# awslabs/crowd-coachable-recommendations

Measured on AMD Instinct MI355X. Metric: queries/sec, exhaustive inner-product top-100 retrieval (NQ-shaped 2,681,468 x 768 bf16 corpus), higher is better.
Workload: dtype bf16

## Files before the change

crowd-coachable-recommendations_amd/ccrec_amd/_lib.py:

```python
import ctypes
import os

_HERE = os.path.dirname(os.path.abspath(__file__))
LIB_PATH = os.path.join(os.path.dirname(_HERE), "lib", "libccr_hip.so")

CCR_OK = 0
CCR_ERR_INVALID, CCR_ERR_HIP, CCR_ERR_WORKSPACE, CCR_ERR_BLOCK_ID = -1, -2, -3, -4
DTYPE_F32, DTYPE_F16, DTYPE_BF16 = 0, 1, 2
SEARCH_DEFAULT, SEARCH_FORCE_DENSE, SEARCH_FORCE_FUSED, SEARCH_ASYNC = 0, 1, 2, 4
SCORES_CANONICAL, SCORES_MFMA = 0, 1

EXPORTS = [
    "ccr_last_error", "ccr_version", "ccr_pack_bf16", "ccr_pack_bf16_ex", "ccr_meanpool_pack_bf16", "ccr_meanpool_pack_bf16_ex", "ccr_index_create",
    "ccr_index_create_with_norms", "ccr_index_destroy",
    "ccr_index_rows", "ccr_index_dim", "ccr_search_workspace_bytes", "ccr_search", "ccr_search_last_stats",
    "ccr_merge_topk", "ccr_merge_topk_strided", "ccr_apply_block", "ccr_inbatch_ce_workspace_bytes", "ccr_inbatch_ce_fwd", "ccr_inbatch_ce_bwd", "ccr_inbatch_ce_bwd_dev", "ccr_rank_metrics",
    "ccr_search_finish", "ccr_scores", "ccr_search_blocked_workspace_bytes", "ccr_search_blocked",
    "ccr_search_sparse_prior_workspace_bytes", "ccr_search_sparse_prior", "ccr_colsum_bf16", "ccr_meanpool_bwd", "ccr_bm25_index_create", "ccr_bm25_index_destroy", "ccr_bm25_search_workspace_bytes",
    "ccr_bm25_search", "ccr_pack_bf16_padded", "ccr_shard_message_bytes", "ccr_search_shard", "ccr_shard_message_fill", "ccr_merge_shard_messages",
    "ccr_attention_bf16", "ccr_add_layernorm", "ccr_meanpool_pack_bf16_packed", "ccr_embed_layernorm", "ccr_gelu_bf16",
    "ccr_attention_half", "ccr_add_layernorm_half", "ccr_embed_layernorm_half", "ccr_gelu_half", "ccr_merge_short_lists",
    "ccr_bm25_search_workspace_bytes_k", "ccr_bm25_search_last_stats", "ccr_bm25_index_set_idf", "ccr_inbatch_pack3_bf16", "ccr_inbatch_ce_fwd_f32",
    "ccr_search_stream_wait_main_pass", "ccr_pool_ce_workspace_bytes", "ccr_pool_ce_fwd", "ccr_pool_ce_fwd_f32", "ccr_pool_ce_bwd_dev",
    "ccr_bpr_sample", "ccr_bpr_frozen_workspace_bytes", "ccr_bpr_frozen_fwd", "ccr_bpr_frozen_bwd_dev",
    "ccr_attention_fwd_train_half", "ccr_attention_bwd_workspace_bytes", "ccr_attention_bwd_half", "ccr_add_layernorm_bwd_half", "ccr_gelu_bwd_half",
    "ccr_dropout_bits_rows", "ccr_dropout_bits_attention", "ccr_dropout_apply", "ccr_attention_fwd_train_drop_half", "ccr_attention_bwd_drop_half",
    "ccr_add_layernorm_drop_half", "ccr_add_layernorm_bwd_drop_half",
]

MIN_VERSION = 101
BPR_VERSION = 102
ENCODER_TRAIN_VERSION = 103
ENCODER_DROPOUT_VERSION = 104

SHARD_HEADER_BYTES = 32
SHARD_MAGIC = 0x4D524343


class ShardHeader(ctypes.Structure):
    _fields_ = [("magic", ctypes.c_uint32), ("n_flagged", ctypes.c_uint32), ("k_valid", ctypes.c_uint32),
                ("n_covered", ctypes.c_uint32), ("row_offset", ctypes.c_int64), ("n_rows", ctypes.c_int64)]


class SearchStats(ctypes.Structure):
    _fields_ = [("path", ctypes.c_int32), ("n_fallback", ctypes.c_int32), ("sample_tiles", ctypes.c_int32),
                ("ranges", ctypes.c_int32), ("cap", ctypes.c_int32), ("sublists", ctypes.c_int32),
                ("n_candidates", ctypes.c_int64), ("ms_sample", ctypes.c_float), ("ms_threshold", ctypes.c_float),
                ("ms_main", ctypes.c_float), ("ms_select", ctypes.c_float), ("ms_fallback", ctypes.c_float),
                ("ms_total", ctypes.c_float), ("n_retried", ctypes.c_int32), ("n_dense", ctypes.c_int32),
                ("main_launches", ctypes.c_int32), ("opt_rank", ctypes.c_int32), ("main_tile_queries", ctypes.c_int32),
                ("skipped_tiles", ctypes.c_int32)]


class CcrError(RuntimeError):
    pass


_lib = None


def load():
    global _lib
    if _lib is not None:
        return _lib
    if not os.path.isfile(LIB_PATH):
        raise CcrError(f"{LIB_PATH} not built: run `python -c 'import __graft_entry__ as g; g.build()'` "
# ... 18 lines not shown
    lib.ccr_meanpool_pack_bf16_ex.argtypes = [vp, i32, vp, vp, vp, vp, vp, i32, i32, i32, i32, vp]
    lib.ccr_index_create.argtypes = [vp, i64, i32, i64, vp, ctypes.POINTER(vp)]
    lib.ccr_index_destroy.argtypes = [vp]
    lib.ccr_index_rows.argtypes = [vp]
    lib.ccr_index_rows.restype = i64
    lib.ccr_index_dim.argtypes = [vp]
    lib.ccr_search_workspace_bytes.argtypes = [vp, i32, i32]
    lib.ccr_search_workspace_bytes.restype = sz
    lib.ccr_search.argtypes = [vp, vp, i32, i32, vp, vp, vp, sz, i32, vp]
    lib.ccr_search_last_stats.argtypes = [vp, ctypes.POINTER(SearchStats)]
    lib.ccr_merge_topk.argtypes = [vp, vp, i32, i32, i32, vp, vp, vp]
    lib.ccr_merge_topk_strided.argtypes = [vp, vp, i64, i64, i32, i32, i32, vp, vp, vp]
    lib.ccr_apply_block.argtypes = [vp, vp, i32, i32, vp, vp, i64, vp, vp, i32, vp]
    lib.ccr_inbatch_ce_workspace_bytes.argtypes = [i32, i32]
    lib.ccr_inbatch_ce_workspace_bytes.restype = sz
    lib.ccr_inbatch_ce_fwd.argtypes = [vp, vp, vp, i32, i32, f32, vp, vp, vp, sz, vp]
    lib.ccr_inbatch_ce_bwd.argtypes = [vp, vp, vp, vp, i32, i32, f32, f32, vp, vp, vp, vp, sz, vp]
    lib.ccr_inbatch_ce_bwd_dev.argtypes = [vp, vp, vp, vp, i32, i32, f32, vp, vp, vp, vp, vp, sz, vp]
    lib.ccr_inbatch_pack3_bf16.argtypes = [vp, vp, vp, i32, i32, vp, vp]
    lib.ccr_inbatch_ce_fwd_f32.argtypes = [vp, vp, vp, i32, i32, f32, vp, vp, vp, vp, sz, vp]
    lib.ccr_pool_ce_workspace_bytes.argtypes = [i32, i32, i32]
    lib.ccr_pool_ce_workspace_bytes.restype = sz
    lib.ccr_pool_ce_fwd.argtypes = [vp, vp, vp, vp, i32, i32, i32, f32, vp, vp, vp, sz, vp]
    lib.ccr_pool_ce_fwd_f32.argtypes = [vp, vp, vp, vp, i32, i32, i32, f32, vp, vp, vp, vp, sz, vp]
    lib.ccr_pool_ce_bwd_dev.argtypes = [vp, vp, vp, vp, vp, i32, i32, i32, f32, vp, vp, vp, vp, vp, sz, vp]
    lib.ccr_bpr_sample.argtypes = [vp, i32, i32, i64, vp, vp, vp, f32, vp, vp, i32, vp, i32, vp, vp]
    lib.ccr_bpr_frozen_workspace_bytes.argtypes = [i32, i32, i32]
    lib.ccr_bpr_frozen_workspace_bytes.restype = sz
    lib.ccr_bpr_frozen_fwd.argtypes = [vp, i64, i32, vp, vp, f32, vp, vp, vp, vp, i32, i32, vp, vp, sz, vp]
    lib.ccr_bpr_frozen_bwd_dev.argtypes = [vp, i64, i32, vp, vp, f32, vp, vp, vp, vp, i32, i32, vp, vp, vp, vp, vp, sz, vp]
    lib.ccr_rank_metrics.argtypes = [vp, i32, i32, vp, vp, vp, i32, vp, vp, vp]
    lib.ccr_search_finish.argtypes = [vp]
    lib.ccr_search_stream_wait_main_pass.argtypes = [vp, vp]
    lib.ccr_scores.argtypes = [vp, vp, i32, i32, vp, vp]
    lib.ccr_search_blocked_workspace_bytes.argtypes = [vp, i32, i32, vp]
    lib.ccr_search_blocked_workspace_bytes.restype = sz
    lib.ccr_search_blocked.argtypes = [vp, vp, i32, i32, vp, vp, vp, vp, vp, sz, i32, vp]
    lib.ccr_search_sparse_prior_workspace_bytes.argtypes = [vp, i32, i32, vp]
    lib.ccr_search_sparse_prior_workspace_bytes.restype = sz
    lib.ccr_search_sparse_prior.argtypes = [vp, vp, i32, i32, vp, vp, vp, vp, vp, vp, sz, i32, vp]
    lib.ccr_colsum_bf16.argtypes = [vp, i64, i32, vp, vp]
    lib.ccr_meanpool_bwd.argtypes = [vp, vp, vp, i32, i32, i32, i32, vp]
    lib.ccr_bm25_index_create.argtypes = [vp, vp, vp, vp, i64, i64, ctypes.c_double, ctypes.POINTER(vp)]
    lib.ccr_bm25_index_destroy.argtypes = [vp]
    lib.ccr_bm25_search_workspace_bytes.argtypes = [vp, i32, i32]
    lib.ccr_bm25_search_workspace_bytes.restype = sz
    lib.ccr_bm25_search_workspace_bytes_k.argtypes = [vp, i32, i32, i32]
    lib.ccr_bm25_search_workspace_bytes_k.restype = sz
    lib.ccr_bm25_search_last_stats.argtypes = [vp, vp]
    lib.ccr_bm25_index_set_idf.argtypes = [vp, vp, vp, vp]
    lib.ccr_bm25_search.argtypes = [vp, vp, vp, vp, i32, i32, vp, vp, vp, sz, vp]
    lib.ccr_pack_bf16_padded.argtypes = [vp, i64, i32, vp, i32, vp, vp, i32, vp]
    lib.ccr_attention_bf16.argtypes = [vp, vp, vp, vp, i32, i32, i32, i32, ctypes.c_float, vp]
    lib.ccr_add_layernorm.argtypes = [vp, vp, vp, vp, ctypes.c_float, vp, vp, i64, i32, vp]
    lib.ccr_embed_layernorm.argtypes = [vp, i64, vp, i64, vp, i64, vp, vp, vp, vp, vp, ctypes.c_float, vp, vp, i64, i32, vp]
    lib.ccr_gelu_bf16.argtypes = [vp, vp, i64, vp]
    lib.ccr_attention_half.argtypes = [vp, vp, vp, vp, i32, i32, i32, i32, ctypes.c_float, i32, vp]
    lib.ccr_add_layernorm_half.argtypes = [vp, vp, vp, vp, ctypes.c_float, vp, vp, i64, i32, i32, vp]
    lib.ccr_embed_layernorm_half.argtypes = [vp, i64, vp, i64, vp, i64, vp, vp, vp, vp, vp, ctypes.c_float, vp, vp, i64, i32, i32, vp]
    lib.ccr_gelu_half.argtypes = [vp, vp, i64, i32, vp]
    lib.ccr_attention_fwd_train_half.argtypes = [vp, vp, vp, vp, vp, i32, i32, i32, i32, ctypes.c_float, i32, vp]
    lib.ccr_attention_bwd_workspace_bytes.argtypes = [i32, i32, i32]
    lib.ccr_attention_bwd_workspace_bytes.restype = sz
    lib.ccr_attention_bwd_half.argtypes = [vp, vp, vp, vp, vp, vp, vp, i32, i32, i32, i32, ctypes.c_float, i32, vp, sz, vp]
    lib.ccr_add_layernorm_bwd_half.argtypes = [vp, vp, vp, ctypes.c_float, vp, vp, vp, vp, vp, i64, i32, i32, vp, sz, vp]
    lib.ccr_gelu_bwd_half.argtypes = [vp, vp, vp, i64, i32, vp]
# ... 30 lines not shown
```

crowd-coachable-recommendations_amd/ccrec_amd/ops.py:

```python
import contextlib
import ctypes

import torch

from . import _lib

_DTYPES = {torch.float32: _lib.DTYPE_F32, torch.float16: _lib.DTYPE_F16, torch.bfloat16: _lib.DTYPE_BF16}


def require_gpu():
    if not torch.cuda.is_available():
        raise _lib.CcrError("ccrec_amd needs a ROCm GPU (torch.cuda.is_available() is False); there is no CPU fallback")
    return _lib.load()


def _stream(t):
    return ctypes.c_void_p(torch.cuda.current_stream(t.device).cuda_stream)


def _ptr(t):
    return ctypes.c_void_p(t.data_ptr()) if t is not None else None


_NO_SWITCH = contextlib.nullcontext()
# ... 697 lines not shown
        return scores, ids

    def search_sparse_prior(self, queries_bf16, k, prior_ptr, prior_idx, prior_val, flags=_lib.SEARCH_DEFAULT):
        q, ptr, idx = self._special_args(queries_bf16, prior_ptr, prior_idx)
        val = torch.as_tensor(prior_val, dtype=torch.float64).to(q.device).contiguous()
        assert val.numel() == idx.numel()
        n_q = q.shape[0]
        scores = torch.empty(n_q, k, dtype=torch.float64, device=q.device)
        ids = torch.empty(n_q, k, dtype=torch.int64, device=q.device)
        if n_q == 0:
            return scores, ids
        if n_q > MAX_QUERIES_PER_SEARCH:
            for lo in range(0, n_q, MAX_QUERIES_PER_SEARCH):
                hi = min(n_q, lo + MAX_QUERIES_PER_SEARCH)
                a, b = int(ptr[lo]), int(ptr[hi])
                s_part, i_part = self.search_sparse_prior(q[lo:hi], k, ptr[lo:hi + 1] - a, idx[a:b], val[a:b], flags)
                scores[lo:hi], ids[lo:hi] = s_part, i_part
            return scores, ids
        pp = ctypes.c_void_p(ptr.data_ptr())
        need = int(self._lib.ccr_search_sparse_prior_workspace_bytes(self._h, n_q, k, pp))
        if need == 0:
            raise _lib.CcrError("ccr_search_sparse_prior: " + self._lib.ccr_last_error().decode("utf-8", "replace"))
        ws = self._special_ws(need)
        with _on(q):
            _lib.check(self._lib.ccr_search_sparse_prior(self._h, _ptr(q), n_q, k, pp, _ptr(idx), _ptr(val), _ptr(scores),
                                                         _ptr(ids), _ptr(ws), ws.numel(), int(flags), _stream(q)),
                       "ccr_search_sparse_prior")
        return scores, ids

    def last_stats(self):
        st = _lib.SearchStats()
        _lib.check(self._lib.ccr_search_last_stats(self._h, ctypes.byref(st)), "ccr_search_last_stats")
        return {f: getattr(st, f) for f, _ in st._fields_}

    def scores(self, queries_bf16, mode="canonical"):
        q = queries_bf16.contiguous()
        assert q.is_cuda and q.dtype == torch.bfloat16 and q.dim() == 2 and q.shape[1] == self.dim
        out = torch.empty(q.shape[0], self.n_rows, dtype=torch.float32, device=q.device)
        if q.shape[0] == 0:
            return out
        m = {"canonical": _lib.SCORES_CANONICAL, "mfma": _lib.SCORES_MFMA}[mode]
        with _on(q):
            _lib.check(self._lib.ccr_scores(self._h, _ptr(q), q.shape[0], m, _ptr(out), _stream(q)), "ccr_scores")
        return out


def _rank_strided(t):
    return t.dim() == 3 and t.stride(2) == 1 and t.stride(1) == t.shape[2] and t.stride(0) >= t.shape[1] * t.shape[2]


def merge_topk(scores, ids):
    lib = require_gpu()
    assert scores.is_cuda and scores.dtype == torch.float32 and ids.dtype == torch.int64 and scores.shape == ids.shape
    if not _rank_strided(scores):
        scores = scores.contiguous()
    if not _rank_strided(ids):
        ids = ids.contiguous()
    R, n_q, k = scores.shape
    os_ = torch.empty(n_q, k, dtype=torch.float32, device=scores.device)
    oi = torch.empty(n_q, k, dtype=torch.int64, device=scores.device)
    with _on(scores):
        _lib.check(lib.ccr_merge_topk_strided(_ptr(scores), _ptr(ids), scores.stride(0), ids.stride(0), R, n_q, k, _ptr(os_),
                                              _ptr(oi), _stream(scores)), "ccr_merge_topk")
    return os_, oi


# ... 347 lines not shown
```

crowd-coachable-recommendations_amd/csrc/ccr_api.hip:

```cpp
#include <stdarg.h>
#include <stdlib.h>
#include <string.h>

#include <math.h>

#include <algorithm>
#include <mutex>
#include <vector>

#include "ccr_index.h"
#include "ccr_narrow.h"
#include "ccr_topk_device.h"

namespace ccr {

static thread_local char g_err[512] = "";
void set_error(const char *fmt, ...) {
    va_list ap;
    va_start(ap, fmt);
    vsnprintf(g_err, sizeof(g_err), fmt, ap);
    va_end(ap);
}

static int env_int(const char *name, int dflt) {
    const char *e = getenv(name);
    return e ? atoi(e) : dflt;
}

Knobs read_knobs() {
    Knobs kn;
    kn.qgroups = env_int("CCR_QGROUPS", 0);
    kn.progressive = env_int("CCR_PROGRESSIVE", 1);
    kn.max_phases = env_int("CCR_PHASES", 3);
    kn.mfma16 = env_int("CCR_MFMA16", -1);
    kn.sample_div = env_int("CCR_SAMPLE_DIV", 0);
    kn.max_lists = env_int("CCR_MAX_LISTS", 0);
    kn.ranges = env_int("CCR_RANGES", 0);
    kn.optimistic = env_int("CCR_OPTIMISTIC", -1);
    kn.opt_rank = env_int("CCR_OPT_RANK", 0);
    kn.narrow = env_int("CCR_NARROW", -1);
    kn.wide = env_int("CCR_WIDE", -1);
    kn.skip_sampled = env_int("CCR_SKIP_SAMPLED", -1);
    kn.skip_list = env_int("CCR_SKIP_LIST", 1);
    kn.narrow_grid = env_int("CCR_NARROW_GRID", 0);
    kn.narrow_groups = env_int("CCR_NARROW_GROUPS", NARROW_MAX_GROUPS);
    return kn;
}

static int pick_qgroups(int qblocks, int dim, const Knobs &kn, int tile_q = TILE_Q) {
    {
        const int v = kn.qgroups;
        if ((v == 1 || v == 2 || v == 4 || v == 8) && qblocks % v == 0) return v;
    }
    const size_t block_bytes = (size_t)tile_q * dim * 2;
    int best = 1;
    for (int gq = 1; gq <= NUM_XCD; gq *= 2) {
        if (qblocks % gq) continue;
        best = gq;
        if ((size_t)(qblocks / gq) * block_bytes <= (size_t)3 << 20) break;
    }
    return best;
}

static inline int64_t round_up(int64_t v, int64_t m) { return (v + m - 1) / m * m; }

static int best_sample_ranges(int64_t n_vt, int qblocks, int qgroups, int grid) {
    const int nrc = NUM_XCD / qgroups, qb_per = qblocks / qgroups, per_x = std::max(1, grid / NUM_XCD);
    int best_r = NUM_XCD;
    double best = 1e300;
    const int64_t r_max = round_up(std::min<int64_t>(n_vt, 1024), NUM_XCD);
    std::vector<double> load((size_t)per_x);
    for (int64_t R = NUM_XCD; R <= r_max; R += NUM_XCD) {
        double worst = 0.0;
        for (int rc = 0; rc < nrc; ++rc) {
            std::fill(load.begin(), load.end(), 0.0);
            const int64_t items = R / nrc * qb_per;
            for (int64_t item = 0; item < items; ++item) {
                const int64_t r = rc + nrc * (item / qb_per);
                const int64_t ntile = (n_vt - r + R - 1) / R;
                if (ntile > 0) load[(size_t)(item % per_x)] += (double)ntile + 0.15;
            }
            worst = std::max(worst, *std::max_element(load.begin(), load.end()));
        }
        if (worst < best - 1e-9) {
            best = worst;
            best_r = (int)R;
        }
    }
    return best_r;
}

constexpr size_t DENSE_SCRATCH_TARGET = (size_t)1 << 30;

struct MainPassChoice {
// ... 157 lines not shown
                            narrow_lds_bytes(nqt, dim) <= (size_t)160 * 1024 && (ngroups == 1 || num_cu >= 16);
        p.narrow = narrow ? nqt : 0;
        p.narrow_groups = narrow ? ngroups : 1;
        p.tile_q = TILE_Q;
        p.main_qblocks = p.qblocks;
        if (!narrow && p.mfma16 && dim % 32 == 0 && kn.wide != 0) {
            const int wb = (n_q + WIDE_Q - 1) / WIDE_Q;
            const double per_xcd = (double)(wb / pick_qgroups(wb, dim, kn, WIDE_Q)) * WIDE_Q * dim * 2.0;
            const double per_flop = per_xcd <= 3.2 * 1048576.0 ? 0.95 : (per_xcd <= 5.5 * 1048576.0 ? 0.97 : 1.04);
            if (kn.wide == 1 || (double)wb * WIDE_Q * per_flop < (double)p.qblocks * TILE_Q) {
                p.tile_q = WIDE_Q;
                p.main_qblocks = wb;
                p.nq_pad = (int)round_up(std::max<int64_t>(n_q, (int64_t)wb * WIDE_Q), TILE_Q);
                p.qblocks = p.nq_pad / TILE_Q;
                p.qgroups = pick_qgroups(p.qblocks, dim, kn);
            }
        }
        p.main_qgroups = pick_qgroups(p.main_qblocks, dim, kn, p.tile_q);
        MainPassChoice choice = choose_main_pass(p, k, sample, sample_alt, sample_big, kn, narrow);
        if (choice.opt_rank > 0 && may_skip_sampled(p, choice.sample, narrow, kn)) {
            const MainPassChoice skipped = choose_main_pass(p, k, sample, sample_alt, sample_big, kn, narrow, choice.sample);
            if (skipped.skip) choice = skipped;
        }
        sample = choice.sample;
        const int64_t R = choice.ranges;
        p.sample_tiles = (int)sample;
        p.sample_stride = std::max<int64_t>(1, p.full_tiles / sample);
        p.sample_ranges = best_sample_ranges(sample, p.qblocks, p.qgroups, p.grid);
        p.ranges = (int)R;
        p.item_a = choice.item_a;
        p.item_b = choice.item_b;
        p.opt_rank = choice.opt_rank;
        p.skip_sampled = (p.opt_rank > 0 && !p.narrow) ? choice.skip : 0;
        if (p.skip_sampled) {
            const double join_rows = 256.0 * (double)choice.sample * (1.0 - pow(1.0 - std::min(1.0, (double)k / (double)n_rows), 16.0));
            const double need = (double)k + (double)(k / 4) + 1.5 * join_rows + TILE_DOCS + 16;
            const double saved = 0.5 * (double)choice.sample * p.main_qblocks * (p.tile_q == WIDE_Q ? 1.37 : 1.0) / (double)p.grid;
            const bool pays = 0.065 * join_rows * ((double)p.nq_pad / 3584.0) < saved;
            if (need > 8192.0 || (kn.skip_sampled < 0 && !pays))
                p.skip_sampled = 0;
            else
                p.rescore_cap = std::min(8192, std::max(p.rescore_cap, pow2_ceil((int)need)));
        }
        const int nrc_p = NUM_XCD / p.main_qgroups, qb_per_p = p.main_qblocks / p.main_qgroups;
        const int64_t RA = p.item_a ? std::min<int64_t>(R, (int64_t)nrc_p * ((p.item_a + qb_per_p - 1) / qb_per_p)) : 0;
        const int64_t RB = p.item_b ? std::min<int64_t>(R, (int64_t)nrc_p * ((p.item_b + qb_per_p - 1) / qb_per_p)) : 0;
        const double ratio = (double)p.tiles / (double)sample;
        const double expect = (double)k * ratio * 1.3 + 64.0;
        const double fs = 1.0 / ratio, nlists = (double)R * p.sublists;
        const double xk = 1.25 * ((double)k + 4.75 * sqrt((double)k) + 8.0) / (double)k;
        const int64_t tile_rows = TILE_DOCS / p.sublists;
        const double xr = p.opt_rank ? 1.25 * ((double)p.opt_rank + 4.75 * sqrt((double)p.opt_rank) + 8.0) / (double)p.opt_rank : 0.0;
        auto cap_for = [&](double g) -> int {
            const double mean = p.opt_rank ? xr * std::max((double)p.opt_rank / fs, (double)k) / nlists : xk * (double)k / (g * nlists);
            const int64_t c = (int64_t)(mean + 6.0 * sqrt(mean)) + 16 + tile_rows;
            return (int)round_up(std::min<int64_t>(std::max<int64_t>(c, 16), 8192), 4);
        };
        const double fa = p.item_a ? (double)(p.item_a / qb_per_p) * nrc_p / (double)R : 0.0;
        const double fb = p.item_b ? std::max(0.0, (double)(p.item_b / qb_per_p) * nrc_p / (double)R - fa) : 0.0;
        const double upd_compact = std::min(32768.0, std::max(4096.0, 8.0 * pow2_ceil(k)));
        auto seen = [&](double g, double found) { return found > upd_compact ? g * upd_compact / found : g; };
        const double found_a = (double)k * fa / fs;
        CandLayout &L = p.cand;
        memset(&L, 0, sizeof(L));
        const int seg_end_v[3] = {RA ? (int)RA : (int)R, RB > RA ? (int)RB : (int)R, (int)R};
        int64_t recs = 0;
// ... 121 lines not shown
int slab_take(int device, uint32_t **out, volatile uint32_t **host_out) {
    std::lock_guard<std::mutex> lock(g_slab_mutex);
    CCR_REQUIRE(device >= 0 && device < MAX_DEVICES, "device ordinal %d out of range", device);
    Slab &sl = g_slabs[device];
    if (!sl.base) {
        CCR_HIP_CHECK(hipMalloc((void **)&sl.base, (size_t)SLAB_SLOTS * SLAB_SLOT_BYTES));
        if (hipHostMalloc((void **)&sl.host, (size_t)SLAB_SLOTS * SLAB_HOST_BYTES, hipHostMallocDefault) != hipSuccess) {
            (void)hipFree(sl.base);
            sl.base = nullptr;
            set_error("ccr_index_create: hipHostMalloc of the pinned flag lines failed");
            return CCR_ERR_HIP;
        }
        for (int i = SLAB_SLOTS - 1; i >= 0; --i) sl.free_slots.push_back(i);
    }
    if (sl.free_slots.empty()) {
        set_error("ccr_index_create: more than %d live indices on device %d", SLAB_SLOTS, device);
        return CCR_ERR_INVALID;
    }
    *out = reinterpret_cast<uint32_t *>(sl.base + (size_t)sl.free_slots.back() * SLAB_SLOT_BYTES);
    *host_out = reinterpret_cast<volatile uint32_t *>(sl.host + (size_t)sl.free_slots.back() * SLAB_HOST_BYTES);
    sl.free_slots.pop_back();
    return CCR_OK;
}

void slab_give(int device, uint32_t *p) {
    if (!p || device < 0 || device >= MAX_DEVICES) return;
    std::lock_guard<std::mutex> lock(g_slab_mutex);
    Slab &sl = g_slabs[device];
    sl.free_slots.push_back((int)((reinterpret_cast<char *>(p) - sl.base) / SLAB_SLOT_BYTES));
}
}

extern "C" const char *ccr_last_error(void) { return g_err; }
extern "C" int ccr_version(void) { return 104; }

extern "C" int ccr_index_destroy(ccr_index *ix);

namespace {
struct CachedBlock {
    void *p;
    size_t bytes;
};
std::vector<CachedBlock> g_blocks[MAX_DEVICES];
constexpr size_t BLOCK_CACHE_ENTRIES = 8;

int block_take(int device, size_t bytes, void **out, size_t *got) {
    CCR_REQUIRE(device >= 0 && device < MAX_DEVICES, "device ordinal %d out of range", device);
    bytes = (bytes + 4095) / 4096 * 4096;
    {
        std::lock_guard<std::mutex> lock(g_slab_mutex);
        auto &v = g_blocks[device];
        for (size_t i = 0; i < v.size(); ++i)
            if (v[i].bytes >= bytes && v[i].bytes <= 2 * bytes) {
                *out = v[i].p;
                *got = v[i].bytes;
                v.erase(v.begin() + i);
                return CCR_OK;
            }
    }
    CCR_HIP_CHECK(hipMalloc(out, bytes));
    *got = bytes;
    return CCR_OK;
}

void block_give(int device, void *p, size_t bytes) {
    if (!p) return;
    void *drop = nullptr;
// ... 84 lines not shown
    block_give(ix->device, ix->row_norm_own, ix->row_bytes);
    if (ix->have_events)
        for (int i = 0; i < EV_COUNT; ++i)
            if (ix->ev[i]) (void)hipEventDestroy(ix->ev[i]);
    delete ix;
    return CCR_OK;
}

extern "C" int64_t ccr_index_rows(const ccr_index *ix) { return ix ? ix->n_rows : -1; }
extern "C" int ccr_index_dim(const ccr_index *ix) { return ix ? ix->dim : -1; }

extern "C" size_t ccr_search_workspace_bytes(const ccr_index *ix, int n_q, int k) {
    if (!ix || n_q <= 0 || k <= 0) return 0;
    Plan a = make_plan(ix->n_rows, ix->dim, n_q, k, CCR_SEARCH_DEFAULT, ix->num_cu, ix->knobs);
    Plan b = make_plan(ix->n_rows, ix->dim, n_q, k, CCR_SEARCH_FORCE_DENSE, ix->num_cu, ix->knobs);
    Plan c = make_plan(ix->n_rows, ix->dim, n_q, k, CCR_SEARCH_FORCE_FUSED, ix->num_cu, ix->knobs);
    return std::max({a.total, b.total, c.total}) + 256;
}

extern "C" int ccr_search_stream_wait_main_pass(const ccr_index *ix, void *stream) {
    CCR_REQUIRE(ix, "ccr_search_stream_wait_main_pass: null index");
    if (!ix->main_pass_recorded) return CCR_OK;
    CCR_HIP_CHECK(hipStreamWaitEvent((hipStream_t)stream, ix->ev[EV_MAIN_END], 0));
    return CCR_OK;
}

extern "C" int ccr_search_last_stats(const ccr_index *ix, ccr_search_stats *stats) {
    CCR_REQUIRE(ix && stats, "ccr_search_last_stats: null pointer");
    CCR_REQUIRE(!ix->pending.active, "ccr_search_last_stats: an asynchronous search is pending (call ccr_search_finish first)");
    *stats = ix->stats;
    return CCR_OK;
}

static int dense_for_list(const ccr_index *ix, const uint16_t *Q, const uint32_t *d_qlist, int n, int k, float *scratch, int64_t rows_per_chunk,
                          float *out_scores, int64_t *out_ids, hipStream_t s) {
    for (int lo = 0; lo < n; lo += (int)rows_per_chunk) {
        const int m = std::min<int64_t>(rows_per_chunk, n - lo);
        int rc = launch_dense_scores(ix->D, ix->n_rows, ix->dim, Q, d_qlist ? d_qlist + lo : nullptr, lo, m, nullptr, scratch, s);
        if (rc != CCR_OK) return rc;
        rc = launch_dense_select(scratch, ix->n_rows, k, d_qlist ? d_qlist + lo : nullptr, lo, m, nullptr, ix->id_out, out_scores, out_ids, s);
        if (rc != CCR_OK) return rc;
    }
    return CCR_OK;
}

static bool margin_path_ok(const ccr_index *ix, int k) { return ix->dim % 8 == 0 && k <= MAX_K; }
static int64_t tiles_of(const ccr_index *ix) { return (ix->n_rows + TILE_DOCS - 1) / TILE_DOCS; }

static GemmArgs gemm_args(const ccr_index *ix, const uint16_t *Q, int n_q, int nq_pad) {
    GemmArgs g;
    memset(&g, 0, sizeof(g));
    g.D = ix->D;
    g.n_rows = ix->n_rows;
    g.dim = ix->dim;
    g.Q = Q;
    g.n_q = n_q;
    g.nq_pad = nq_pad;
    g.qblocks = nq_pad / TILE_Q;
    g.item_end = INT32_MAX;
    return g;
}

static GemmArgs filter_args(const ccr_index *ix, const Plan &p, const SearchWs &w, const uint16_t *Q, int n_q, int nq_pad, int qblocks,
                            int qgroups, const float *thr, const float *cq, const CandLayout &lay) {
    GemmArgs g = gemm_args(ix, Q, n_q, nq_pad);
    g.qblocks = qblocks;
// ... 12 lines not shown

static int store_scores(const ccr_index *ix, const uint16_t *Q, int n_q, int ranges, float *out, int64_t pitch, hipStream_t s) {
    GemmArgs g = gemm_args(ix, Q, n_q, (int)round_up(n_q, TILE_Q));
    g.n_vt = tiles_of(ix);
    g.tile_stride = 1;
    g.ranges = ranges;
    g.qgroups = 1;
    g.store = out;
    g.store_pitch = pitch;
    return launch_gemm(g, ix->knobs.mfma16 != 0 ? MAIN_16X16 : MAIN_32X32, EPI_STORE, std::max(NUM_XCD, ix->num_cu / NUM_XCD * NUM_XCD), s);
}

static int margin_for_rows(const ccr_index *ix, const uint16_t *Qc, const float *hint, const uint32_t *out_rows, int n, int k, float *scratch,
                           size_t scratch_bytes, float *out_scores, int64_t *out_ids, uint32_t *flag_count, uint32_t *flag_list, hipStream_t s) {
    const int64_t pitch = round_up(ix->n_rows, 4);
    int64_t chunk = (int64_t)(scratch_bytes / ((size_t)pitch * 4));
    CCR_REQUIRE(chunk >= 1, "margin path: no room for one score row");
    if (chunk > TILE_Q) chunk = chunk / TILE_Q * TILE_Q;
    const int ranges = (int)round_up(std::min<int64_t>(std::max<int64_t>(1, tiles_of(ix) / 4), 1024), NUM_XCD);
    for (int lo = 0; lo < n; lo += (int)chunk) {
        const int m = std::min<int64_t>(chunk, n - lo);
        const uint16_t *Q = Qc + (int64_t)lo * ix->dim;
        int rc = store_scores(ix, Q, m, ranges, scratch, pitch, s);
        if (rc != CCR_OK) return rc;
        rc = launch_margin_select(scratch, pitch, ix->n_rows, k, ix->dim, Q, ix->D, ix->tile_norm, ix->row_norm, ix->dmax_bits,
                                  hint ? hint + lo : nullptr, out_rows ? out_rows + lo : nullptr, lo, m, ix->id_out, out_scores, out_ids, flag_count, flag_list, s);
        if (rc != CCR_OK) return rc;
    }
    return CCR_OK;
}

static int run_main_pass(const ccr_index *ix, const Plan &p, const SearchWs &w, const uint16_t *Q, int n_q, int k, hipStream_t s) {
    GemmArgs gm = filter_args(ix, p, w, Q, n_q, p.nq_pad, p.main_qblocks, p.main_qgroups, w.thr, w.cq, p.cand);
    if (p.skip_sampled) {
        gm.n_vt = p.tiles - p.sample_tiles;
        gm.skip_stride = (int)p.sample_stride;
        gm.skip_count = p.sample_tiles;
    }
    const int nrc = NUM_XCD / gm.qgroups, qb_per = gm.qblocks / gm.qgroups, items = p.ranges / nrc * qb_per;
    const int bounds[4] = {0, p.item_a, p.item_b, items};
    int done = 0, updates = 0, prev_full = 0, prev_part = 0, prev_blocks = 0;
    for (int ph = 1; ph < 4; ++ph) {
        if (bounds[ph] <= done) continue;
        if (done > 0) {
            const int rl_full = done / qb_per, part = done % qb_per;
            const int full = rl_full * nrc * p.sublists, partial = part ? (rl_full + 1) * nrc * p.sublists : 0;
            const bool more = bounds[ph] < items && ph < 3;
            const int rc = launch_threshold_update(w.cand, w.cnt, full, partial, part, prev_full, prev_part, prev_blocks, qb_per, p.sublists, n_q,
                                                   p.nq_pad, p.cand, k, w.cq, ix->tile_norm, p.item_b ? w.top : nullptr, updates > 0, more, w.thr, s, p.tile_q);
            if (rc != CCR_OK) return rc;
            prev_full = full;
            prev_part = partial;
            prev_blocks = part;
            ++updates;
        }
        gm.item_begin = done;
        gm.item_end = bounds[ph];
        const MainKernel kind = p.tile_q == WIDE_Q ? MAIN_WIDE : p.mfma16 ? MAIN_16X16 : MAIN_32X32;
        const int rc = launch_gemm(gm, kind, EPI_FILTER, p.grid, s);
        if (rc != CCR_OK) return rc;
        done = bounds[ph];
    }
    return CCR_OK;
}

static int run_narrow_pass(const ccr_index *ix, const Plan &p, const SearchWs &w, const uint16_t *Q, int n_q, hipStream_t s) {
// ... 346 lines not shown
```

crowd-coachable-recommendations_amd/csrc/ccr_common.h:

```cpp
#pragma once
#include <hip/hip_runtime.h>
#include <stdint.h>
#include <stdio.h>

#include "ccr_retrieval.h"

namespace ccr {

void set_error(const char *fmt, ...);

#define CCR_HIP_CHECK(expr)                                                                   \
    do {                                                                                      \
        hipError_t _e = (expr);                                                               \
        if (_e != hipSuccess) {                                                               \
            ccr::set_error("%s failed: %s (%s:%d)", #expr, hipGetErrorString(_e), __FILE__, __LINE__); \
            return CCR_ERR_HIP;                                                               \
        }                                                                                     \
    } while (0)

#define CCR_REQUIRE(cond, ...)            \
    do {                                  \
        if (!(cond)) {                    \
            ccr::set_error(__VA_ARGS__);  \
            return CCR_ERR_INVALID;       \
// ... 15 lines not shown
constexpr int TILE_K = 32;
constexpr int GEMM_THREADS = 512;
constexpr int GROUPS_PER_TILE = 16;
constexpr int MAX_K = 4096;
constexpr uint32_t FLAG_DENSE = 0x80000000u;
constexpr int NUM_XCD = 8;

struct CandLayout {
    int nseg;
    int seg_end[3];
    int cap[3];
    long long base[3];
};
__host__ __device__ __forceinline__ void cand_segment(const CandLayout &L, int r, int &cap, int &r0, long long &base) {
    const int g = (r >= L.seg_end[0] ? 1 : 0) + (r >= L.seg_end[1] ? 1 : 0);
    r0 = g ? L.seg_end[g - 1] : 0;
    cap = L.cap[g];
    base = L.base[g];
}
__host__ __device__ __forceinline__ long long cand_sublist(const CandLayout &L, int r, int q, int s, int nq_pad, int sp, int &cap) {
    const int g = (r >= L.seg_end[0] ? 1 : 0) + (r >= L.seg_end[1] ? 1 : 0);
    const int r0 = g ? L.seg_end[g - 1] : 0;
    cap = L.cap[g];
    return L.base[g] + (((long long)(r - r0) * nq_pad + q) * sp) * (long long)cap + s;
}

struct Plan {
    int fused;
    int nq_pad;
    int qblocks;
    int tile_q;
    int main_qblocks;
    int main_qgroups;
    int64_t tiles;
    int64_t full_tiles;
    int sample_tiles;
    int64_t sample_stride;
    int sample_ranges;
    int ranges;
    int item_a;
    int item_b;
    int opt_rank;
    int skip_sampled;
    int qgroups;
    int cap;
    CandLayout cand;
    int grid;
    int rescore_cap;
    int rescore_regular;
    int select_compact;
    int mfma16;
    int sublists;
    int narrow;
    int narrow_groups;
    int first_nsub;
    int first_sp;
    CandLayout first_lay;
    int64_t cand_recs;
    size_t off_qnorm, off_thr, off_gmax, off_cnt, off_cand, off_flag, off_dense, off_retry, off_top, off_safe, total;
    int64_t dense_rows_per_chunk;
};

__host__ __device__ __forceinline__ int64_t unsampled_tile(int64_t v, int s, int n) {
    if (s == 0) return v;
    const uint32_t u = (uint32_t)v, d = (uint32_t)(s - 1);
    return u < (uint32_t)n * d ? (int64_t)(u + u / d + 1u) : v + n;
}

enum { EPI_FILTER = 0, EPI_GMAX = 1, EPI_STORE = 2 };

struct GemmArgs {
    const uint16_t *D;
    int64_t n_rows;
    int dim;
    const uint16_t *Q;
    int n_q;
    int nq_pad;
    int qblocks;
    int64_t n_vt;
    int64_t tile_stride;
    int ranges;
    int skip_stride, skip_count;
    int qgroups;
    int item_begin, item_end;
    const float *thr;
    const float *cq;
    const float *tile_norm;
    uint2 *cand;
    uint32_t *cnt;
    CandLayout lay;
    float *gmax;
    float *store;
    int64_t store_pitch;
};


__device__ __forceinline__ float bf16_bits_to_f32(uint16_t h) { return __uint_as_float(((uint32_t)h) << 16); }

__device__ __forceinline__ uint32_t f32_orderable(float f) {
    uint32_t u = __float_as_uint(f);
    return (u & 0x80000000u) ? ~u : (u | 0x80000000u);
}
__device__ __forceinline__ float orderable_to_f32(uint32_t u) {
    return __uint_as_float((u & 0x80000000u) ? (u & 0x7fffffffu) : ~u);
}

constexpr int64_t ID_LOCAL_U32 = INT64_MIN;
__device__ __forceinline__ void store_id(int64_t *out_ids, int64_t pos, int64_t id_offset, uint32_t row) {
    if (id_offset == ID_LOCAL_U32)
        reinterpret_cast<uint32_t *>(out_ids)[pos] = row;
    else
        out_ids[pos] = id_offset + (int64_t)row;
}

__host__ __device__ __forceinline__ float mfma_gamma(int dim) { return (float)dim * 1.1920929e-7f * 1.02f; }

// ... 2 lines not shown
```

crowd-coachable-recommendations_amd/csrc/ccr_fused.hip:

```cpp
#include <stdlib.h>

#include <mutex>
#include <set>
#include <type_traits>
#include <utility>

#include "ccr_gemm_common.h"
#include "ccr_index.h"
#include "ccr_topk_device.h"

namespace ccr {

__device__ __attribute__((aligned(16))) uint32_t g_zero_chunk[4];

__device__ __forceinline__ float load_uniform_f32(const float *p) {
    float v;
    asm volatile("s_load_dword %0, %1, 0x0\n\ts_waitcnt lgkmcnt(0)" : "=s"(v) : "s"(p) : "memory");
    return v;
}

template <int N>
__device__ __forceinline__ void wait_vm() {
    asm volatile("s_waitcnt vmcnt(%0)" ::"n"(N) : "memory");
}

typedef float f32x4v __attribute__((ext_vector_type(4)));

__device__ __forceinline__ float max4_asm(const f32x4v &c) {
    float m;
    asm("v_max3_f32 %0, %1, %2, %3\n\tv_max_f32 %0, %0, %4" : "=&v"(m) : "v"(c[0]), "v"(c[1]), "v"(c[2]), "v"(c[3]));
    return m;
}
__device__ __forceinline__ float max3_asm(float a, float b, float c) {
    float m;
    asm("v_max3_f32 %0, %1, %2, %3" : "=v"(m) : "v"(a), "v"(b), "v"(c));
    return m;
}

__device__ __forceinline__ int64_t real_tile(const GemmArgs &a, int64_t vt) {
    return a.skip_stride ? unsampled_tile(vt, a.skip_stride, a.skip_count) : vt * a.tile_stride;
}

struct ItemWalk {
    int jx, step, qg, rc, nrc, qb_per, end;
    __device__ __forceinline__ explicit ItemWalk(const GemmArgs &a) {
        const int xcd = blockIdx.x & (NUM_XCD - 1);
        jx = blockIdx.x >> 3;
        step = gridDim.x >> 3;
        qg = xcd % a.qgroups;
        rc = xcd / a.qgroups;
        nrc = NUM_XCD / a.qgroups;
        qb_per = a.qblocks / a.qgroups;
        const int count_x = (a.ranges / nrc) * qb_per;
        end = a.item_end < count_x ? a.item_end : count_x;
    }
    __device__ __forceinline__ int first(const GemmArgs &a) const { return a.item_begin + jx; }
    __device__ __forceinline__ int64_t item(const GemmArgs &a, int i, int &r, int &qb) const {
        const int rl = i / qb_per;
        const int b = qg * qb_per + i % qb_per;
        const int ri = rc + nrc * rl;
        const int64_t ntile = (a.n_vt - ri + a.ranges - 1) / a.ranges;
        r = ri;
        qb = b;
        return ntile;
    }
};


struct Mfma32 {
    typedef f32x16 Acc;
    static constexpr int TILE = 32, REGS = 16, DT = 4, QT = 2, SUBLISTS = 4;
    struct Frags { bf16x8 a[2][4], b[2][2]; };

    static __device__ __forceinline__ int src_swizzle(int row) { return (row >> 2) & 3; }

    int a_base, b_base, cofs[2];
    __device__ __forceinline__ Mfma32(int lane, int wd, int wq) {
        const int swz = (lane >> 2) & 3;
#pragma unroll
        for (int ks = 0; ks < 2; ++ks) cofs[ks] = (((2 * ks + (lane >> 5)) ^ swz) << 4);
        a_base = (wd * 128 + (lane & 31)) * 64;
        b_base = SUB_Q_REGION + (wq * 64 + (lane & 31)) * 64;
    }
    __device__ __forceinline__ void read(const char *buf, Frags &f) const {
#pragma unroll
        for (int ks = 0; ks < 2; ++ks) {
#pragma unroll
            for (int dt = 0; dt < 4; ++dt) f.a[ks][dt] = *reinterpret_cast<const bf16x8 *>(buf + a_base + dt * 2048 + cofs[ks]);
#pragma unroll
            for (int qt = 0; qt < 2; ++qt) f.b[ks][qt] = *reinterpret_cast<const bf16x8 *>(buf + b_base + qt * 2048 + cofs[ks]);
        }
    }
    static __device__ __forceinline__ void mma(Acc (&acc)[4][2], const Frags &f, bool first) {
        if (first) {
            const f32x16 z = {0.f, 0.f, 0.f, 0.f, 0.f, 0.f, 0.f, 0.f, 0.f, 0.f, 0.f, 0.f, 0.f, 0.f, 0.f, 0.f};
#pragma unroll
            for (int dt = 0; dt < 4; ++dt)
// ... 1514 lines not shown
```

crowd-coachable-recommendations_amd/csrc/ccr_index.h:

```cpp
#pragma once
#include "ccr_common.h"

namespace ccr {

struct Knobs {
    int qgroups;
    int progressive;
    int max_phases;
    int mfma16;
    int sample_div;
    int ranges;
    int optimistic;
    int opt_rank;
    int max_lists;
    int narrow;
    int narrow_grid;
    int skip_sampled;
    int skip_list;
    int wide;
    int narrow_groups;
};
Knobs read_knobs();

constexpr int FALLBACK_ROWS = 16;

Plan make_plan(int64_t n_rows, int dim, int n_q, int k, int flags, int num_cu, const Knobs &kn);

struct Bump {
    size_t off;
    size_t take(size_t bytes) { const size_t o = off; off = (off + bytes + 255) / 256 * 256; return o; }
};

struct SearchWs {
    float *qnorm, *thr, *cq, *gmax;
    uint32_t *cnt;
    uint2 *cand;
    uint32_t *flag_count, *flag_list;
    unsigned long long *stat_cand;
    uint32_t *top;
    float *thr_safe, *cq_safe, *dense;
    uint32_t *glist;
    uint16_t *Q2;
    float *thr2, *cq2;
    uint32_t *retry_list, *dense_list, *counts, *flag2, *list_b, *list_c;
    size_t cand_bytes, dense_bytes, retry_bytes, total;
};
SearchWs search_ws(const Plan &p, int64_t n_rows, int dim, int n_q, int k, char *base);
inline int skip_list_cap(int opt_rank) { return 2 * opt_rank + 30; }

enum MainKernel { MAIN_32X32, MAIN_16X16, MAIN_WIDE };
int launch_gemm(const GemmArgs &a, MainKernel kind, int epi, int grid, hipStream_t s);
// ... 73 lines not shown
```

include/ccr_retrieval.h:

```cpp
#ifndef CCR_RETRIEVAL_H
#define CCR_RETRIEVAL_H

#include <stddef.h>
#include <stdint.h>

#ifdef __cplusplus
extern "C" {
#endif

#define CCR_OK 0
#define CCR_ERR_INVALID (-1)
#define CCR_ERR_HIP (-2)
#define CCR_ERR_WORKSPACE (-3)
#define CCR_ERR_BLOCK_ID (-4)

#define CCR_DTYPE_F32 0
#define CCR_DTYPE_F16 1
#define CCR_DTYPE_BF16 2

#define CCR_SEARCH_DEFAULT 0
#define CCR_SEARCH_FORCE_DENSE 1
#define CCR_SEARCH_FORCE_FUSED 2
#define CCR_SEARCH_ASYNC 4

// ... 81 lines not shown
int ccr_dropout_bits_attention(uint32_t *keep_q, uint32_t *keep_k, const int32_t *seq_start, const int32_t *seq_len, int64_t n_tokens,
                               int n_seq, int n_heads, int max_len, uint64_t seed, uint32_t stream_id, double p, void *stream);
int ccr_dropout_apply(const float *x, const uint32_t *bits, float inv_keep, float *out_f32, uint16_t *out_half, int64_t rows, int dim,
                      int half_dtype, void *stream);
int ccr_attention_fwd_train_drop_half(const uint16_t *qkv, const int32_t *seq_start, const int32_t *seq_len, uint16_t *out, float *lse,
                                      const uint32_t *keep_q, float inv_keep, int n_seq, int n_heads, int max_len, int pad_len,
                                      float scale, int half_dtype, void *stream);
int ccr_attention_bwd_drop_half(const uint16_t *qkv, const uint16_t *out, const float *lse, const uint16_t *d_out,
                                const int32_t *seq_start, const int32_t *seq_len, const uint32_t *keep_q, const uint32_t *keep_k,
                                float inv_keep, uint16_t *d_qkv, int n_seq, int n_heads, int max_len, int pad_len, float scale,
                                int half_dtype, void *workspace, size_t workspace_bytes, void *stream);
int ccr_add_layernorm_drop_half(const uint16_t *x_half, const uint32_t *bits, float inv_keep, const float *residual, const float *gamma,
                                const float *beta, float eps, float *out_f32, uint16_t *out_half, int64_t rows, int dim, int half_dtype,
                                void *stream);
int ccr_add_layernorm_bwd_drop_half(const uint16_t *x_half, const uint32_t *bits, float inv_keep, const float *residual,
                                    const float *gamma, float eps, const float *d_y, float *d_res, uint16_t *d_x, float *d_gamma,
                                    float *d_beta, int64_t rows, int dim, int half_dtype, void *workspace, size_t workspace_bytes,
                                    void *stream);

int ccr_index_create(const uint16_t *D_bf16, int64_t n_rows, int dim, int64_t global_row_offset, void *stream,
                     ccr_index **out);
int ccr_index_create_with_norms(const uint16_t *D_bf16, int64_t n_rows, int dim, int64_t global_row_offset,
                                const float *row_norm_bounds, void *stream, ccr_index **out);
int ccr_index_destroy(ccr_index *index);
int64_t ccr_index_rows(const ccr_index *index);
int ccr_index_dim(const ccr_index *index);

size_t ccr_search_workspace_bytes(const ccr_index *index, int n_q, int k);
int ccr_search(ccr_index *index, const uint16_t *Q_bf16, int n_q, int k, float *out_scores, int64_t *out_ids,
               void *workspace, size_t ws_bytes, int flags, void *stream);
int ccr_search_finish(ccr_index *index);
int ccr_search_last_stats(const ccr_index *index, ccr_search_stats *stats );
int ccr_search_stream_wait_main_pass(const ccr_index *index, void *stream);

int ccr_scores(const ccr_index *index, const uint16_t *Q_bf16, int n_q, int mode, float *out, void *stream);

size_t ccr_search_blocked_workspace_bytes(const ccr_index *index, int n_q, int k, const int64_t *block_ptr_host);
int ccr_search_blocked(ccr_index *index, const uint16_t *Q_bf16, int n_q, int k, const int64_t *block_ptr_host,
                       const int64_t *block_idx, float *out_scores, int64_t *out_ids, void *workspace, size_t ws_bytes,
                       int flags, void *stream);

size_t ccr_search_sparse_prior_workspace_bytes(const ccr_index *index, int n_q, int k, const int64_t *prior_ptr_host);
int ccr_search_sparse_prior(ccr_index *index, const uint16_t *Q_bf16, int n_q, int k, const int64_t *prior_ptr_host,
                            const int64_t *prior_idx, const double *prior_val, double *out_scores, int64_t *out_ids,
                            void *workspace, size_t ws_bytes, int flags, void *stream);

int ccr_colsum_bf16(const uint16_t *X, int64_t rows, int dim, double *out , void *stream);

int ccr_merge_topk(const float *scores, const int64_t *ids, int R, int n_q, int k, float *out_scores,
                   int64_t *out_ids, void *stream);
int ccr_merge_topk_strided(const float *scores, const int64_t *ids, int64_t score_rank_stride, int64_t id_rank_stride,
                           int R, int n_q, int k, float *out_scores, int64_t *out_ids, void *stream);

#define CCR_SHARD_MAGIC 0x4d524343u
typedef struct ccr_shard_header {
    uint32_t magic;
    uint32_t n_flagged;
    uint32_t k_valid;
    uint32_t n_covered;
    int64_t row_offset;
    int64_t n_rows;
} ccr_shard_header;
size_t ccr_shard_message_bytes(int n_q, int k);
int ccr_search_shard(ccr_index *index, const uint16_t *Q_bf16, int n_q, int k, void *message, void *workspace, size_t ws_bytes,
                     int flags, void *stream);
int ccr_shard_message_fill(void *message, int n_q, int k, int k_valid, const float *scores, const int64_t *ids, int64_t row_offset,
// ... 65 lines not shown
```

Baseline: 259,200.

## Split query blocks unevenly across XCD groups when qblocks is not divisible

Adds a qsplit mode to the fused main pass. When the number of query blocks does not divide evenly across the XCD groups, each group owns its base share and the remainder blocks are spread across work items. The split is picked so that the per-XCD query footprint falls into a smaller cache-size class than the equal-group plan. This is meant to keep each XCD's query working set cache-resident and to balance work. The cost is a more complex work-item index mapping in the kernel and a heuristic that may not fire for a given batch size.

Result: faster. 262,200 (median of 6 runs) (+1.1%).

```diff
diff --git a/crowd-coachable-recommendations_amd/ccrec_amd/_lib.py b/crowd-coachable-recommendations_amd/ccrec_amd/_lib.py
--- a/crowd-coachable-recommendations_amd/ccrec_amd/_lib.py
+++ b/crowd-coachable-recommendations_amd/ccrec_amd/_lib.py
@@ -25,13 +25,14 @@
     "ccr_bpr_sample", "ccr_bpr_frozen_workspace_bytes", "ccr_bpr_frozen_fwd", "ccr_bpr_frozen_bwd_dev",
     "ccr_attention_fwd_train_half", "ccr_attention_bwd_workspace_bytes", "ccr_attention_bwd_half", "ccr_add_layernorm_bwd_half", "ccr_gelu_bwd_half",
     "ccr_dropout_bits_rows", "ccr_dropout_bits_attention", "ccr_dropout_apply", "ccr_attention_fwd_train_drop_half", "ccr_attention_bwd_drop_half",
-    "ccr_add_layernorm_drop_half", "ccr_add_layernorm_bwd_drop_half",
+    "ccr_add_layernorm_drop_half", "ccr_add_layernorm_bwd_drop_half", "ccr_search_last_main_split",
 ]
 
 MIN_VERSION = 101
 BPR_VERSION = 102
 ENCODER_TRAIN_VERSION = 103
 ENCODER_DROPOUT_VERSION = 104
+QSPLIT_VERSION = 105
 
 SHARD_HEADER_BYTES = 32
 SHARD_MAGIC = 0x4D524343
@@ -116,6 +117,7 @@
     lib.ccr_rank_metrics.argtypes = [vp, i32, i32, vp, vp, vp, i32, vp, vp, vp]
     lib.ccr_search_finish.argtypes = [vp]
     lib.ccr_search_stream_wait_main_pass.argtypes = [vp, vp]
+    lib.ccr_search_last_main_split.argtypes = [vp]
     lib.ccr_scores.argtypes = [vp, vp, i32, i32, vp, vp]
     lib.ccr_search_blocked_workspace_bytes.argtypes = [vp, i32, i32, vp]
     lib.ccr_search_blocked_workspace_bytes.restype = sz
diff --git a/crowd-coachable-recommendations_amd/ccrec_amd/ops.py b/crowd-coachable-recommendations_amd/ccrec_amd/ops.py
--- a/crowd-coachable-recommendations_amd/ccrec_amd/ops.py
+++ b/crowd-coachable-recommendations_amd/ccrec_amd/ops.py
@@ -753,6 +753,9 @@
         st = _lib.SearchStats()
         _lib.check(self._lib.ccr_search_last_stats(self._h, ctypes.byref(st)), "ccr_search_last_stats")
         return {f: getattr(st, f) for f, _ in st._fields_}
+
+    def last_main_split(self):
+        return int(self._lib.ccr_search_last_main_split(self._h))
 
     def scores(self, queries_bf16, mode="canonical"):
         q = queries_bf16.contiguous()
diff --git a/crowd-coachable-recommendations_amd/csrc/ccr_api.hip b/crowd-coachable-recommendations_amd/csrc/ccr_api.hip
--- a/crowd-coachable-recommendations_amd/csrc/ccr_api.hip
+++ b/crowd-coachable-recommendations_amd/csrc/ccr_api.hip
@@ -42,6 +42,7 @@
     kn.wide = env_int("CCR_WIDE", -1);
     kn.skip_sampled = env_int("CCR_SKIP_SAMPLED", -1);
     kn.skip_list = env_int("CCR_SKIP_LIST", 1);
+    kn.qsplit = env_int("CCR_QSPLIT", -1);
     kn.narrow_grid = env_int("CCR_NARROW_GRID", 0);
     kn.narrow_groups = env_int("CCR_NARROW_GROUPS", NARROW_MAX_GROUPS);
     return kn;
@@ -60,6 +61,22 @@
         if ((size_t)(qblocks / gq) * block_bytes <= (size_t)3 << 20) break;
     }
     return best;
+}
+
+static int footprint_class(double bytes) { return bytes <= 3.2 * 1048576.0 ? 0 : (bytes <= 5.5 * 1048576.0 ? 1 : 2); }
+
+static int pick_qsplit(int qblocks, int equal_groups, int dim, int tile_q, const Knobs &kn) {
+    if (kn.qsplit == 0) return 0;
+    const int v = kn.qgroups;
+    if (v == 2 || v == 4 || v == 8) return qblocks % v ? v : 0;
+    const double block_bytes = (double)tile_q * dim * 2.0;
+    const int equal_class = footprint_class((double)(qblocks / equal_groups) * block_bytes);
+    for (int G = 2; G <= NUM_XCD; G *= 2)
+        if (qblocks % G && footprint_class((double)(qblocks / G + qblocks % G) * block_bytes) < equal_class) return G;
+    if (kn.qsplit == 1)
+        for (int G = 2; G <= NUM_XCD; G *= 2)
+            if (qblocks % G) return G;
+    return 0;
 }
 
 static inline int64_t round_up(int64_t v, int64_t m) { return (v + m - 1) / m * m; }
@@ -283,6 +300,7 @@
         p.item_b = choice.item_b;
         p.opt_rank = choice.opt_rank;
         p.skip_sampled = (p.opt_rank > 0 && !p.narrow) ? choice.skip : 0;
+        p.main_qsplit = (!p.narrow && p.item_a == 0 && p.item_b == 0) ? pick_qsplit(p.main_qblocks, p.main_qgroups, dim, p.tile_q, kn) : 0;
         if (p.skip_sampled) {
             const double join_rows = 256.0 * (double)choice.sample * (1.0 - pow(1.0 - std::min(1.0, (double)k / (double)n_rows), 16.0));
             const double need = (double)k + (double)(k / 4) + 1.5 * join_rows + TILE_DOCS + 16;
@@ -470,7 +488,7 @@
 }
 
 extern "C" const char *ccr_last_error(void) { return g_err; }
-extern "C" int ccr_version(void) { return 104; }
+extern "C" int ccr_version(void) { return 105; }
 
 extern "C" int ccr_index_destroy(ccr_index *ix);
 
@@ -621,6 +639,11 @@
     return CCR_OK;
 }
 
+extern "C" int ccr_search_last_main_split(const ccr_index *ix) {
+    if (!ix || ix->plan_nq <= 0 || !ix->plan.fused) return 0;
+    return ix->plan.main_qsplit;
+}
+
 static int dense_for_list(const ccr_index *ix, const uint16_t *Q, const uint32_t *d_qlist, int n, int k, float *scratch, int64_t rows_per_chunk,
                           float *out_scores, int64_t *out_ids, hipStream_t s) {
     for (int lo = 0; lo < n; lo += (int)rows_per_chunk) {
@@ -699,6 +722,7 @@
 
 static int run_main_pass(const ccr_index *ix, const Plan &p, const SearchWs &w, const uint16_t *Q, int n_q, int k, hipStream_t s) {
     GemmArgs gm = filter_args(ix, p, w, Q, n_q, p.nq_pad, p.main_qblocks, p.main_qgroups, w.thr, w.cq, p.cand);
+    gm.qsplit = p.main_qsplit;
     if (p.skip_sampled) {
         gm.n_vt = p.tiles - p.sample_tiles;
         gm.skip_stride = (int)p.sample_stride;
diff --git a/crowd-coachable-recommendations_amd/csrc/ccr_common.h b/crowd-coachable-recommendations_amd/csrc/ccr_common.h
--- a/crowd-coachable-recommendations_amd/csrc/ccr_common.h
+++ b/crowd-coachable-recommendations_amd/csrc/ccr_common.h
@@ -71,6 +71,7 @@
     int tile_q;
     int main_qblocks;
     int main_qgroups;
+    int main_qsplit;
     int64_t tiles;
     int64_t full_tiles;
     int sample_tiles;
@@ -106,6 +107,35 @@
     return u < (uint32_t)n * d ? (int64_t)(u + u / d + 1u) : v + n;
 }
 
+__host__ __device__ __forceinline__ int64_t main_item(int i, int xcd, int qblocks, int qgroups, int qsplit, int ranges, int64_t n_vt, int &r,
+                                                      int &qb) {
+    const int groups = qsplit ? qsplit : qgroups, g = xcd % groups, rc = xcd / groups, nrc = NUM_XCD / groups;
+    const int base = qblocks / groups;
+    int rl, b;
+    if (qsplit == 0) {
+        rl = i / base;
+        b = g * base + i % base;
+    } else {
+        const int rem = qblocks - base * groups;
+        const int period = i / qblocks, o = i - period * qblocks;
+        int row = g, k = o - g * base;
+        if (k < 0) {
+            row = o / base;
+            k = o - row * base;
+        } else if (k >= base + rem) {
+            row = (o - rem) / base;
+            k = o - rem - row * base;
+        }
+        rl = period * groups + row;
+        b = k >= base ? groups * base + (k - base) : g * base + k;
+    }
+    const int ri = rc + nrc * rl;
+    const int64_t ntile = (n_vt - ri + ranges - 1) / ranges;
+    r = ri;
+    qb = b;
+    return ntile;
+}
+
 enum { EPI_FILTER = 0, EPI_GMAX = 1, EPI_STORE = 2 };
 
 struct GemmArgs {
@@ -121,6 +151,7 @@
     int ranges;
     int skip_stride, skip_count;
     int qgroups;
+    int qsplit;
     int item_begin, item_end;
     const float *thr;
     const float *cq;
diff --git a/crowd-coachable-recommendations_amd/csrc/ccr_fused.hip b/crowd-coachable-recommendations_amd/csrc/ccr_fused.hip
--- a/crowd-coachable-recommendations_amd/csrc/ccr_fused.hip
+++ b/crowd-coachable-recommendations_amd/csrc/ccr_fused.hip
@@ -42,27 +42,17 @@
 }
 
 struct ItemWalk {
-    int jx, step, qg, rc, nrc, qb_per, end;
+    int jx, step, xcd, end;
     __device__ __forceinline__ explicit ItemWalk(const GemmArgs &a) {
-        const int xcd = blockIdx.x & (NUM_XCD - 1);
+        xcd = blockIdx.x & (NUM_XCD - 1);
         jx = blockIdx.x >> 3;
         step = gridDim.x >> 3;
-        qg = xcd % a.qgroups;
-        rc = xcd / a.qgroups;
-        nrc = NUM_XCD / a.qgroups;
-        qb_per = a.qblocks / a.qgroups;
-        const int count_x = (a.ranges / nrc) * qb_per;
+        const int count_x = (a.ranges / NUM_XCD) * a.qblocks;
         end = a.item_end < count_x ? a.item_end : count_x;
     }
     __device__ __forceinline__ int first(const GemmArgs &a) const { return a.item_begin + jx; }
     __device__ __forceinline__ int64_t item(const GemmArgs &a, int i, int &r, int &qb) const {
-        const int rl = i / qb_per;
-        const int b = qg * qb_per + i % qb_per;
-        const int ri = rc + nrc * rl;
-        const int64_t ntile = (a.n_vt - ri + a.ranges - 1) / a.ranges;
-        r = ri;
-        qb = b;
-        return ntile;
+        return main_item(i, xcd, a.qblocks, a.qgroups, a.qsplit, a.ranges, a.n_vt, r, qb);
     }
 };
 
diff --git a/crowd-coachable-recommendations_amd/csrc/ccr_index.h b/crowd-coachable-recommendations_amd/csrc/ccr_index.h
--- a/crowd-coachable-recommendations_amd/csrc/ccr_index.h
+++ b/crowd-coachable-recommendations_amd/csrc/ccr_index.h
@@ -17,6 +17,7 @@
     int narrow_grid;
     int skip_sampled;
     int skip_list;
+    int qsplit;
     int wide;
     int narrow_groups;
 };
diff --git a/include/ccr_retrieval.h b/include/ccr_retrieval.h
--- a/include/ccr_retrieval.h
+++ b/include/ccr_retrieval.h
@@ -137,6 +137,7 @@
 int ccr_search_finish(ccr_index *index);
 int ccr_search_last_stats(const ccr_index *index, ccr_search_stats *stats );
 int ccr_search_stream_wait_main_pass(const ccr_index *index, void *stream);
+int ccr_search_last_main_split(const ccr_index *index);
 
 int ccr_scores(const ccr_index *index, const uint16_t *Q_bf16, int n_q, int mode, float *out, void *stream);
 
```
